# DerEchteKarsten/RayTracer3

Hardware: AMD Instinct MI355X
Metric: Mrays/s (higher is better)
Workload: dtype f32

## Files before the change

### raytracer3_amd/csrc/rt3_kernels.hip

```cpp
#include <hip/hip_fp16.h>
#include <hip/hip_runtime.h>

#include "rt3_device.hpp"
#include "rt3_internal.hpp"

namespace rt3 {

constexpr int kLdsStack = 12;
constexpr uint32_t kTopFlag = 0x40000000u;
constexpr int kSpill = 64 - kLdsStack;
constexpr uint32_t kMaxSteps = 1u << 20;

constexpr uint32_t kEmptySlot = 0xFFFFFFFFu;
constexpr float kTopPadRel = 2.44140625e-4f;

struct Cand {
    float tn;
    uint32_t ref;
};
__device__ __forceinline__ void cswap(Cand& a, Cand& b) {
    bool sw = b.tn < a.tn;
    float ta = a.tn;
    uint32_t ra = a.ref;
    a.tn = sw ? b.tn : a.tn;
// ... 314 lines not shown
                        RT3_REF48(m0, r0)
                        RT3_REF48(m1, r1)
                        RT3_REF48(m2, r2)
                        RT3_REF48(m3, r3)
#undef RT3_REF48
                    } else {
                        r0 = __float_as_uint(q2.z);
                        r1 = __float_as_uint(q2.w);
                        r2 = __float_as_uint(q3.x);
                        r3 = __float_as_uint(q3.y);
                    }
#define RT3_Q(w, b) ((float)(((w) >> (8 * (b))) & 0xFFu))
#define RT3_SLABQ(lx, ly, lz, hx, hy, hz, tn) \
    slab_test_q(__builtin_fmaf(lx, A.x, B.x), __builtin_fmaf(hx, A.x, B.x), __builtin_fmaf(ly, A.y, B.y), __builtin_fmaf(hy, A.y, B.y), \
                __builtin_fmaf(lz, A.z, B.z), __builtin_fmaf(hz, A.z, B.z), tmin, r.best.t, tn)
                    if (LAYOUT == kLayoutWide64Q) {
#define RT3_SLABS(wlo, whi, selp, selq, tn)                                                                                                    \
    (TWO ? slab_test_sorted_pad(__builtin_amdgcn_perm(whi, wlo, selp), __builtin_amdgcn_perm(whi, wlo, selq), A, B, tl_pad, tmin, r.best.t, tn) \
         : slab_test_sorted(__builtin_amdgcn_perm(whi, wlo, selp), __builtin_amdgcn_perm(whi, wlo, selq), A, B, tmin, r.best.t, tn))
                        h0 = RT3_SLABS(w0, w1, r.sel_p0, r.sel_q0, t0) & (r0 != kEmptySlot);
                        h1 = RT3_SLABS(w1, w2, r.sel_p1, r.sel_q1, t1) & (r1 != kEmptySlot);
                        h2 = RT3_SLABS(w3, w4, r.sel_p0, r.sel_q0, t2) & (r2 != kEmptySlot);
                        h3 = RT3_SLABS(w4, w5, r.sel_p1, r.sel_q1, t3) & (r3 != kEmptySlot);
#undef RT3_SLABS
                    } else {
                    h0 = RT3_SLABQ(RT3_Q(w0, 0), RT3_Q(w0, 1), RT3_Q(w0, 2), RT3_Q(w0, 3), RT3_Q(w1, 0), RT3_Q(w1, 1), t0) & (r0 != kEmptySlot);
                    h1 = RT3_SLABQ(RT3_Q(w1, 2), RT3_Q(w1, 3), RT3_Q(w2, 0), RT3_Q(w2, 1), RT3_Q(w2, 2), RT3_Q(w2, 3), t1) & (r1 != kEmptySlot);
                    h2 = RT3_SLABQ(RT3_Q(w3, 0), RT3_Q(w3, 1), RT3_Q(w3, 2), RT3_Q(w3, 3), RT3_Q(w4, 0), RT3_Q(w4, 1), t2) & (r2 != kEmptySlot);
                    h3 = RT3_SLABQ(RT3_Q(w4, 2), RT3_Q(w4, 3), RT3_Q(w5, 0), RT3_Q(w5, 1), RT3_Q(w5, 2), RT3_Q(w5, 3), t3) & (r3 != kEmptySlot);
                    }
#undef RT3_Q
#undef RT3_SLABQ
                } else {
                    r0 = __float_as_uint(q1.z);
                    r1 = __float_as_uint(q3.z);
                    r2 = __float_as_uint(q5.z);
                    r3 = __float_as_uint(q7.z);
                    h0 = slab_test_hw(v3(q0.x, q0.y, q0.z), v3(q0.w, q1.x, q1.y), o, inv, tmin, r.best.t, t0) & (r0 != kEmptySlot);
                    h1 = slab_test_hw(v3(q2.x, q2.y, q2.z), v3(q2.w, q3.x, q3.y), o, inv, tmin, r.best.t, t1) & (r1 != kEmptySlot);
                    h2 = slab_test_hw(v3(q4.x, q4.y, q4.z), v3(q4.w, q5.x, q5.y), o, inv, tmin, r.best.t, t2) & (r2 != kEmptySlot);
                    h3 = slab_test_hw(v3(q6.x, q6.y, q6.z), v3(q6.w, q7.x, q7.y), o, inv, tmin, r.best.t, t3) & (r3 != kEmptySlot);
                }
                Cand c0{h0 ? (ANY ? -t0 : t0) : kInf, h0 ? r0 : kEmptySlot}, c1{h1 ? (ANY ? -t1 : t1) : kInf, h1 ? r1 : kEmptySlot};
                Cand c2{h2 ? (ANY ? -t2 : t2) : kInf, h2 ? r2 : kEmptySlot}, c3{h3 ? (ANY ? -t3 : t3) : kInf, h3 ? r3 : kEmptySlot};
                const uint32_t nh = (uint32_t)h0 + (uint32_t)h1 + (uint32_t)h2 + (uint32_t)h3;
                cswap(c0, c1);
                cswap(c2, c3);
                cswap(c0, c2);
                cswap(c1, c3);
                cswap(c1, c2);
                if (nh > 3) {
                    if (r.sp < kLdsStack) lds[r.sp * kExtendBlock] = c3.ref;
                    else spill[r.sp - kLdsStack] = c3.ref;
                    ++r.sp;
                }
                if (nh > 2) {
                    if (r.sp < kLdsStack) lds[r.sp * kExtendBlock] = c2.ref;
                    else spill[r.sp - kLdsStack] = c2.ref;
                    ++r.sp;
                }
                if (nh > 1) {
                    if (r.sp < kLdsStack) lds[r.sp * kExtendBlock] = c1.ref;
                    else spill[r.sp - kLdsStack] = c1.ref;
                    ++r.sp;
                }
                r.cur = c0.ref;
                pop = nh == 0;
            } else {
                float tn0, tn1;
                uint32_t r0 = __float_as_uint(q3.x), r1 = __float_as_uint(q3.y);
                bool h0 = slab_test_hw(v3(q0.x, q0.y, q0.z), v3(q0.w, q1.x, q1.y), o, inv, tmin, r.best.t, tn0) & (r0 != kEmptySlot);
                bool h1 = slab_test_hw(v3(q1.z, q1.w, q2.x), v3(q2.y, q2.z, q2.w), o, inv, tmin, r.best.t, tn1) & (r1 != kEmptySlot);
                bool near1 = tn1 < tn0;
                if (h0 & h1) {
                    uint32_t far = near1 ? r0 : r1;
                    if (r.sp < kLdsStack) lds[r.sp * kExtendBlock] = far;
                    else spill[r.sp - kLdsStack] = far;
                    ++r.sp;
                }
                r.cur = (h0 & h1) ? (near1 ? r1 : r0) : (h0 ? r0 : r1);
                pop = !(h0 | h1);
            }
        }
        if (pop && !done) {
            if (TWO && tl_bottom && (uint32_t)r.sp == tl_mark) {
                tl_world();
                tl_sels();
            }
            if (r.sp == 0) {
                done = true;
            } else {
                --r.sp;
                if (r.sp < kLdsStack) {
                    r.cur = lds[r.sp * kExtendBlock];
                } else {
                    r.cur = spill[r.sp - kLdsStack];
                    __builtin_amdgcn_sched_barrier(0);
                }
            }
        }
        if (++r.steps >= kMaxSteps) done = true;
        if (done) {
            finish(r.index, r.best, r.cn, r.ct, r.cl, MODE == 2 ? lane_any : MODE == 1, r.pay0, r.pay1, r.pay2, r.pay3);
            busy = false;
        }
        }
    }
}

template <bool COUNT, int LAYOUT>
__global__ __launch_bounds__(kExtendBlock) void k_extend(const float4* __restrict__ nodes, const float4* __restrict__ tris, const float4* __restrict__ top, uint32_t n_top,
                                                         const float* __restrict__ rays, size_t stride,
                                                         const uint32_t* __restrict__ count_ptr, uint32_t count_imm,
                                                         float* __restrict__ hits, uint32_t* __restrict__ cnt_nodes,
                                                         uint32_t* __restrict__ cnt_tris, unsigned long long* __restrict__ totals,
                                                         uint32_t* __restrict__ work_counter, int payload, unsigned long long* __restrict__ lds_total) {
    __shared__ uint32_t stack[kLdsStack * kExtendBlock];
    __shared__ float4 s_top[4 * kTopNodes];
    const bool use_top = load_top(s_top, top, n_top);
    const uint32_t n = count_ptr ? *count_ptr : count_imm;
    unsigned long long tot_n = 0, tot_t = 0, tot_l = 0;
    auto finish = [&](uint32_t i, const Hit& h, uint32_t cn, uint32_t ct, uint32_t cl, bool, float, float, float, float) {
        reinterpret_cast<float4*>(hits)[i] = make_float4(h.t, h.u, h.v, __uint_as_float(h.prim));
        if (COUNT) {
            if (cnt_nodes) cnt_nodes[i] = cn;
            if (cnt_tris) cnt_tris[i] = ct;
            tot_n += cn;
            tot_t += ct;
            tot_l += cl;
        }
    };
    trace_stream<0, COUNT, LAYOUT == kLayoutTwoLevel ? kLayoutWide64Q : LAYOUT, LAYOUT == kLayoutTwoLevel>(nodes, tris, rays, stride, n, work_counter, stack + threadIdx.x, finish, false, nullptr, 0, nullptr, payload != 0, s_top, use_top);
    if (COUNT && totals) {
        atomicAdd(&totals[0], tot_n);
        atomicAdd(&totals[1], tot_t);
        if (lds_total) atomicAdd(lds_total, tot_l);
    }
}

template <bool COUNT, int LAYOUT>
__global__ __launch_bounds__(kExtendBlock) void k_shadow(const float4* __restrict__ nodes, const float4* __restrict__ tris, const float4* __restrict__ top, uint32_t n_top,
                                                         const float* __restrict__ rays, size_t stride,
                                                         const uint32_t* __restrict__ count_ptr, uint32_t count_imm,
                                                         const float* __restrict__ contrib, const uint32_t* __restrict__ pid,
                                                         float* __restrict__ lacc, size_t lstride,
                                                         uint32_t* __restrict__ occluded_out, uint32_t* __restrict__ cnt_nodes,
                                                         uint32_t* __restrict__ cnt_tris, unsigned long long* __restrict__ totals,
                                                         uint32_t* __restrict__ work_counter, unsigned long long* __restrict__ lds_total) {
    __shared__ uint32_t stack[kLdsStack * kExtendBlock];
    __shared__ float4 s_top[4 * kTopNodes];
    const bool use_top = load_top(s_top, top, n_top);
    const uint32_t n = count_ptr ? *count_ptr : count_imm;
    unsigned long long tot_n = 0, tot_t = 0, tot_l = 0;
    trace_stream<1, COUNT, LAYOUT == kLayoutTwoLevel ? kLayoutWide64Q : LAYOUT, LAYOUT == kLayoutTwoLevel>(
        nodes, tris, rays, stride, n, work_counter, stack + threadIdx.x,
        [&](uint32_t i, const Hit& h, uint32_t cn, uint32_t ct, uint32_t cl, bool, float c_r, float c_g, float c_b, float c_pid) {
            if (occluded_out) {
                occluded_out[i] = h.prim != kMiss ? 1u : 0u;
            } else if (h.prim == kMiss) {
                float4* L = reinterpret_cast<float4*>(lacc) + __float_as_uint(c_pid);
                float4 v = *L;
                *L = make_float4(v.x + c_r, v.y + c_g, v.z + c_b, 0.0f);
            }
            if (COUNT) {
                if (cnt_nodes) cnt_nodes[i] = cn;
                if (cnt_tris) cnt_tris[i] = ct;
                tot_n += cn;
                tot_t += ct;
                tot_l += cl;
            }
        },
        occluded_out == nullptr, nullptr, 0, nullptr, false, s_top, use_top, occluded_out == nullptr ? reinterpret_cast<const float2*>(contrib) : nullptr);
    if (COUNT && totals) {
        atomicAdd(&totals[0], tot_n);
        atomicAdd(&totals[1], tot_t);
        if (lds_total) atomicAdd(lds_total, tot_l);
    }
}

template <bool COUNT, int LAYOUT>
__global__ __launch_bounds__(kExtendBlock) void k_trace(const float4* __restrict__ nodes, const float4* __restrict__ tris, const float4* __restrict__ top, uint32_t n_top,
                                                        const float* __restrict__ ext_rays, const float* __restrict__ sh_rays, size_t stride,
                                                        const uint32_t* __restrict__ ext_count, const uint32_t* __restrict__ sh_count,
                                                        float* __restrict__ hits, const float* __restrict__ contrib, float* __restrict__ lacc,
                                                        unsigned long long* __restrict__ totals, uint32_t* __restrict__ work_ext,
                                                        uint32_t* __restrict__ work_sh) {
    __shared__ uint32_t stack[kLdsStack * kExtendBlock];
    __shared__ float4 s_top[4 * kTopNodes];
    const bool use_top = load_top(s_top, top, n_top);
    const uint32_t n_ext = *ext_count, n_sh = *sh_count;
    unsigned long long en = 0, et = 0, sn = 0, stt = 0, el = 0, sl = 0;
    trace_stream<2, COUNT, LAYOUT == kLayoutTwoLevel ? kLayoutWide64Q : LAYOUT, LAYOUT == kLayoutTwoLevel>(
        nodes, tris, ext_rays, stride, n_ext, work_ext, stack + threadIdx.x,
        [&](uint32_t i, const Hit& h, uint32_t cn, uint32_t ct, uint32_t cl, bool any, float c_r, float c_g, float c_b, float c_pid) {
            if (!any) {
                reinterpret_cast<float4*>(hits)[i] = make_float4(h.t, h.u, h.v, __uint_as_float(h.prim));
            } else if (h.prim == kMiss) {
                float4* L = reinterpret_cast<float4*>(lacc) + __float_as_uint(c_pid);
                float4 v = *L;
                *L = make_float4(v.x + c_r, v.y + c_g, v.z + c_b, 0.0f);
            }
            if (COUNT) {
                en += any ? 0u : cn;
                et += any ? 0u : ct;
                sn += any ? cn : 0u;
                stt += any ? ct : 0u;
                el += any ? 0u : cl;
                sl += any ? cl : 0u;
            }
        },
        true, sh_rays, n_sh, work_sh, true, s_top, use_top, reinterpret_cast<const float2*>(contrib));
    if (COUNT && totals) {
        if (blockIdx.x == 0 && threadIdx.x == 0) {
            atomicAdd(&totals[0], (unsigned long long)n_ext);
            atomicAdd(&totals[3], (unsigned long long)n_sh);
        }
        atomicAdd(&totals[1], en);
        atomicAdd(&totals[2], et);
        atomicAdd(&totals[4], sn);
        atomicAdd(&totals[5], stt);
        atomicAdd(&totals[6], el);
        atomicAdd(&totals[7], sl);
    }
}

__global__ void k_raygen(GConstDev g, const uint32_t* __restrict__ pixels, uint32_t npix, float* __restrict__ rays, size_t stride) {
    for (uint32_t i = blockIdx.x * blockDim.x + threadIdx.x; i < npix; i += gridDim.x * blockDim.x) {
        uint32_t xy = pixels[i];
        V3 o, d;
        primary_ray(g, xy & 0xFFFFu, xy >> 16, o, d);
        reinterpret_cast<float4*>(rays)[i] = make_float4(o.x, o.y, o.z, 0.0f);
        reinterpret_cast<float4*>(rays)[stride + i] = make_float4(d.x, d.y, d.z, kBackgroundDepth);
    }
}
__global__ void k_gbuffer(SceneDev sc, const uint32_t* __restrict__ pixels, uint32_t npix, uint32_t width,
                          const float* __restrict__ hits, size_t stride, uint4* __restrict__ gbuffer, float* __restrict__ depth) {
    for (uint32_t i = blockIdx.x * blockDim.x + threadIdx.x; i < npix; i += gridDim.x * blockDim.x) {
        uint32_t xy = pixels[i];
        size_t pi = (size_t)(xy >> 16) * width + (xy & 0xFFFFu);
        const float4 hrec = reinterpret_cast<const float4*>(hits)[i];
        uint32_t prim = __float_as_uint(hrec.w);
        if (prim == kMiss) {
            depth[pi] = kBackgroundDepth;
        } else {
            Surface s = hit_info(sc, prim, hrec.y, hrec.z);
            gbuffer[pi] = gbuffer_pack(s);
            depth[pi] = hrec.x;
        }
    }
}

constexpr int kShadeBlock = 512;
struct BlockAppend {
    uint32_t ext, sh;
};
__device__ __forceinline__ BlockAppend block_append2(bool want_ext, bool want_sh, unsigned long long* pair ,
                                                     uint32_t* lds ) {
    constexpr int kWaves = kShadeBlock / 64;
    const uint32_t lane = __lane_id(), wave = threadIdx.x >> 6;
    const unsigned long long m_ext = __ballot(want_ext), m_sh = __ballot(want_sh);
    if (lane == 0) {
        lds[wave] = (uint32_t)__popcll(m_ext);
        lds[kWaves + 1 + wave] = (uint32_t)__popcll(m_sh);
    }
    __syncthreads();
    if (threadIdx.x == 0) {
        uint32_t te = 0, ts = 0;
#pragma unroll
        for (int w = 0; w < kWaves; w++) {
            uint32_t ce = lds[w], cs = lds[kWaves + 1 + w];
            lds[w] = te;
            lds[kWaves + 1 + w] = ts;
            te += ce;
            ts += cs;
        }
        unsigned long long old = 0ull;
        if (te | ts) old = atomicAdd(pair, (unsigned long long)te | ((unsigned long long)ts << 32));
        lds[kWaves] = (uint32_t)old;
        lds[2 * kWaves + 1] = (uint32_t)(old >> 32);
    }
    __syncthreads();
    const unsigned long long below = (1ull << lane) - 1ull;
    BlockAppend r;
    r.ext = lds[kWaves] + lds[wave] + (uint32_t)__popcll(m_ext & below);
    r.sh = lds[2 * kWaves + 1] + lds[kWaves + 1 + wave] + (uint32_t)__popcll(m_sh & below);
    return r;
}

struct ShadeArgs {
    GConstDev g;
    SceneDev sc;
    const uint32_t* pixels;
    const uint2* pixbn;
    uint32_t npix, width;
    FastDiv npix_div;
    uint32_t s0;
    uint32_t bounce;
    const uint4* gbuffer;
    const float* depth;
    const float* in_rays;
    const float* in_hits;
    const float* in_T;
    const uint32_t* in_count;
    uint32_t n_first;
    float* out_rays;
    float* out_T;
    uint32_t* out_count;
    float* sh_rays;
    float* sh_contrib;
    uint32_t* sh_count;
    float* lacc;
    size_t stride;
};

template <bool FIRST, bool GLDS>
__global__ __launch_bounds__(kShadeBlock) __attribute__((amdgpu_waves_per_eu(6, 6))) void k_shade(ShadeArgs a) {
    __shared__ uint32_t append_lds[2][2 * (kShadeBlock / 64 + 1)];
    __shared__ ShadeGeomDev s_geoms[GLDS ? kShadeGeomsLds : 1];
    if (GLDS) {
        const uint32_t words = (a.sc.n_geoms < kShadeGeomsLds ? a.sc.n_geoms : kShadeGeomsLds) * (uint32_t)(sizeof(ShadeGeomDev) / 4);
        for (uint32_t k = threadIdx.x; k < words; k += kShadeBlock) reinterpret_cast<uint32_t*>(s_geoms)[k] = reinterpret_cast<const uint32_t*>(a.sc.shade_geoms)[k];
        __syncthreads();
    }
    uint32_t parity = 0;
    constexpr uint32_t kMargRows = 2048;
    __shared__ uint32_t s_guide_marg[kMargRows];
    __shared__ float s_cdf_marg[kMargRows + 4];
    const bool marg_in_lds = (a.g.pad[0] & RT3_FLAG_NEE_SKY) && a.sc.sky != nullptr && a.sc.sky_h <= kMargRows;
    if (marg_in_lds) {
        for (uint32_t k = threadIdx.x; k < a.sc.sky_h; k += kShadeBlock) s_guide_marg[k] = a.sc.guide_marg[k];
        for (uint32_t k = threadIdx.x; k < a.sc.sky_h + 4u; k += kShadeBlock) s_cdf_marg[k] = a.sc.cdf_marg[k];
        __syncthreads();
    }
    const float* cdf_marg = marg_in_lds ? s_cdf_marg : a.sc.cdf_marg;
    const uint32_t* guide_marg = marg_in_lds ? s_guide_marg : a.sc.guide_marg;
    const GConstDev& g = a.g;
    const uint32_t flags = g.pad[0], B = g.bounces, b = a.bounce;
    const uint32_t dims = flags ? 8u : 2u;
    const bool nee = (flags & RT3_FLAG_NEE_SKY) && a.sc.sky != nullptr;
    const bool bnz = (flags & RT3_FLAG_BLUENOISE) && a.sc.bluenoise != nullptr;
    const bool spec = (flags & RT3_FLAG_SPECULAR) != 0u;
    const size_t S = a.stride;
    const uint32_t n = FIRST ? a.n_first : *a.in_count;
    const uint32_t n_round = (n + (kShadeBlock - 1)) & ~(uint32_t)(kShadeBlock - 1);
    for (uint32_t i = blockIdx.x * blockDim.x + threadIdx.x; i < n_round; i += gridDim.x * blockDim.x) {
        bool active = i < n;
        uint32_t pid = 0;
        V3 o = v3(0, 0, 0), d = v3(0, 0, 1), T = v3(1, 1, 1);
        float t = 0.0f, pdf_b = 0.0f;
        Surface surf;
        surf.albedo = surf.emissive = v3(0, 0, 0);
        surf.normal = v3(0, 0, 1);
        surf.roughness = 1.0f;
        surf.metalness = 0.0f;
        uint32_t px = 0, py = 0, sample_in_batch = 0, bn = 0;
        HitRecord hrecord;
        hrecord.rec = make_uint4(0u, 0u, 0u, 0u);
        hrecord.prim = 0u;
        float hbu = 0.0f, hbv = 0.0f;
        float4 ro = make_float4(0.0f, 0.0f, 0.0f, 0.0f), rd = make_float4(0.0f, 0.0f, 1.0f, 0.0f);
        if (!FIRST && active) {
            ro = reinterpret_cast<const float4*>(a.in_rays)[i];
            rd = reinterpret_cast<const float4*>(a.in_rays)[S + i];
        }
        if (active) {
            pid = FIRST ? i : __float_as_uint(rd.w);
            sample_in_batch = fast_div(a.npix_div, pid);
            const uint2 pb = a.pixbn[pid - sample_in_batch * a.npix];
            px = pb.x & 0xFFFFu;
            py = pb.x >> 16;
            bn = pb.y;
        }
        if (FIRST) {
            if (active) {
                size_t pi = (size_t)py * a.width + px;
                float d0 = a.depth[pi];
                if (d0 == kBackgroundDepth) {
                    reinterpret_cast<float4*>(a.lacc)[pid] = make_float4(0.0f, 0.0f, 0.0f, 0.0f);
                    active = false;
                } else {
                    surf = gbuffer_unpack(a.gbuffer[pi]);
                    primary_ray(g, px, py, o, d);
                    t = d0;
                }
            }
        } else if (active) {
            o = v3(ro.x, ro.y, ro.z);
            d = v3(rd.x, rd.y, rd.z);
            T = v3(a.in_T[i], a.in_T[S + i], a.in_T[2 * S + i]);
            pdf_b = ro.w;
            const float4 hrec = reinterpret_cast<const float4*>(a.in_hits)[i];
            uint32_t prim = __float_as_uint(hrec.w);
            if (prim == kMiss) {
                if (nee && pdf_b > 0.0f) {
                    float su, sv;
                    direction_to_equirect_uv(d, su, sv);
                    float pl;
                    V3 rad = sky_eval_and_pdf(a.sc, su, sv, pl);
                    float w = pdf_b / (pdf_b + pl);
                    float4* Lp = reinterpret_cast<float4*>(a.lacc) + pid;
                    float4 lv = *Lp;
                    *Lp = make_float4(lv.x + T.x * (rad.x * w), lv.y + T.y * (rad.y * w), lv.z + T.z * (rad.z * w), 0.0f);
                }
                active = false;
            } else {
                t = hrec.x;
                hbu = hrec.y;
                hbv = hrec.z;
                hrecord = hit_fetch(a.sc, prim);
            }
        }
        bool emit_shadow = false, emit_ext = false;
        V3 wl = v3(0, 1, 0), contrib = v3(0, 0, 0), nd = v3(0, 0, 1), Tn = T;
        float pdf_n = 0.0f;
        if (active) {
            uint32_t seed = rng_seed(px, py, g.frame);
            uint32_t sm = a.s0 + sample_in_batch;
            uint32_t base = (sm * B + b) * dims;
            float u0 = uniform_float(seed, base), u1 = uniform_float(seed, base + 1);
            if (bnz) {
                u0 = bluenoise_shift(u0, bn & 0xFFu);
                u1 = bluenoise_shift(u1, (bn >> 8) & 0xFFu);
            }
            V3 rad = v3(0.0f, 0.0f, 0.0f);
            float pl = 0.0f, cosl = 0.0f;
            SkyPick pick;
            pick.u = pick.v = pick.sin_theta = 0.0f;
            pick.x = pick.y = 0;
            if (nee) {
                float ul0 = uniform_float(seed, base + 3), ul1 = uniform_float(seed, base + 4);
                if (bnz) {
                    ul0 = bluenoise_shift(ul0, (bn >> 16) & 0xFFu);
                    ul1 = bluenoise_shift(ul1, (bn >> 24) & 0xFFu);
                }
                pick = sky_sample_direction(a.sc, cdf_marg, guide_marg, ul0, ul1, wl);
            }
            if (!FIRST) {
                if (GLDS) surf = hit_finish(a.sc, s_geoms, hrecord, hbu, hbv);
                else surf = hit_finish(a.sc, a.sc.shade_geoms, hrecord, hbu, hbv);
            }
            V3 N = surf.normal;
            if ((flags & RT3_FLAG_FACEFORWARD) && dot(N, d) > 0.0f) N = neg(N);
            if (nee) {
                cosl = dot(N, wl);
                if (cosl > 0.0f) sky_sample_radiance(a.sc, pick, rad, pl);
            }
            V3 b1, b2;
            build_orthonormal_basis(N, b1, b2);
            V3 wi = v3(0.0f, 0.0f, 1.0f), vop = surf.albedo, wo = v3(0.0f, 0.0f, 1.0f);
            float pdf_s = 0.0f;
            bool valid = true;
            Bsdf bs;
            const bool last = b == B - 1;
            if (spec) {
                bs = bsdf_setup(surf.albedo, surf.roughness, surf.metalness);
                wo = v3(-(d.x * b1.x + d.y * b1.y + d.z * b1.z), -(d.x * b2.x + d.y * b2.y + d.z * b2.z), -(d.x * N.x + d.y * N.y + d.z * N.z));
                if (!last) {
                    float u2 = uniform_float(seed, base + 2);
                    valid = bsdf_sample(bs, wo, u0, u1, u2, wi, vop, pdf_s);
                }
            } else if (!last) {
                wi = diffuse_sample(u0, u1);
                pdf_s = wi.z * kInvPi;
            }
            o = v3(o.x + t * d.x, o.y + t * d.y, o.z + t * d.z);
            if (FIRST) {
                reinterpret_cast<float4*>(a.lacc)[pid] = make_float4(T.x * surf.emissive.x, T.y * surf.emissive.y, T.z * surf.emissive.z, 0.0f);
            } else if (surf.emissive.x != 0.0f || surf.emissive.y != 0.0f || surf.emissive.z != 0.0f) {
                float4* Lp = reinterpret_cast<float4*>(a.lacc) + pid;
                float4 lv = *Lp;
                *Lp = make_float4(lv.x + T.x * surf.emissive.x, lv.y + T.y * surf.emissive.y, lv.z + T.z * surf.emissive.z, 0.0f);
            }
            if (nee) {
                if (cosl > 0.0f && pl > 0.0f) {
                    V3 fv;
                    float scale;
                    if (spec) {
                        float pproj;
                        bsdf_eval(bs, wo, v3(dot(wl, b1), dot(wl, b2), cosl), fv, pproj);
                        float pb = pproj * cosl;
                        scale = (b == B - 1) ? cosl / pl : cosl / (pl + pb);
                    } else {
                        float pb = cosl * kInvPi;
                        fv = surf.albedo;
                        scale = (b == B - 1) ? (cosl * kInvPi) / pl : (cosl * kInvPi) / (pl + pb);
                    }
                    contrib = v3((T.x * fv.x) * (rad.x * scale), (T.y * fv.y) * (rad.y * scale), (T.z * fv.z) * (rad.z * scale));
                    emit_shadow = true;
                }
            }
            if (valid && !last) {
                nd = basis_apply(b1, b2, N, wi);
                pdf_n = pdf_s;
                Tn = T * vop;
                emit_ext = true;
            }
        }
        const BlockAppend slot = block_append2(emit_ext, emit_shadow, reinterpret_cast<unsigned long long*>(a.out_count), append_lds[parity]);
        parity ^= 1u;
        if (emit_shadow) {
            const uint32_t j = slot.sh;
            reinterpret_cast<float4*>(a.sh_rays)[j] = make_float4(o.x, o.y, o.z, contrib.x);
            reinterpret_cast<float4*>(a.sh_rays)[S + j] = make_float4(wl.x, wl.y, wl.z, contrib.y);
            reinterpret_cast<float2*>(a.sh_contrib)[j] = make_float2(contrib.z, __uint_as_float(pid));
        }
        if (emit_ext) {
            const uint32_t j = slot.ext;
            reinterpret_cast<float4*>(a.out_rays)[j] = make_float4(o.x, o.y, o.z, pdf_n);
            reinterpret_cast<float4*>(a.out_rays)[S + j] = make_float4(nd.x, nd.y, nd.z, __uint_as_float(pid));
            a.out_T[j] = Tn.x;
            a.out_T[S + j] = Tn.y;
            a.out_T[2 * S + j] = Tn.z;
        }
    }
}

__global__ void k_accumulate(GConstDev g, const uint32_t* __restrict__ pixels, uint32_t npix, uint32_t width,
                             const float* __restrict__ depth, const float* __restrict__ lacc, size_t stride, uint32_t sb,
                             int first_batch, int last_batch, float* __restrict__ radsum, float4* __restrict__ light,
                             const float4* __restrict__ prev) {
    for (uint32_t i = blockIdx.x * blockDim.x + threadIdx.x; i < npix; i += gridDim.x * blockDim.x) {
        uint32_t xy = pixels[i];
        size_t pi = (size_t)(xy >> 16) * width + (xy & 0xFFFFu);
        if (depth[pi] == kBackgroundDepth) continue;
        float r = first_batch ? 0.0f : radsum[i], gg = first_batch ? 0.0f : radsum[npix + i], bb = first_batch ? 0.0f : radsum[2 * (size_t)npix + i];
        for (uint32_t s = 0; s < sb; s++) {
            size_t p = (size_t)s * npix + i;
            const float4 lv = reinterpret_cast<const float4*>(lacc)[p];
            r += lv.x;
            gg += lv.y;
            bb += lv.z;
        }
        if (!last_batch) {
            radsum[i] = r;
            radsum[npix + i] = gg;
            radsum[2 * (size_t)npix + i] = bb;
        } else {
            float fs = (float)g.samples;
            r = r / fs;
            gg = gg / fs;
            bb = bb / fs;
            if (g.blendfactor >= 1.0f) {
                light[pi] = make_float4(r, gg, bb, 0.0f);
            } else {
                float4 pv = prev[pi];
                float bf = g.blendfactor;
                light[pi] = make_float4(pv.x + (r - pv.x) * bf, pv.y + (gg - pv.y) * bf, pv.z + (bb - pv.z) * bf, 0.0f);
            }
        }
    }
}

__device__ __forceinline__ float agx_contrast(float x) {
    float x2 = x * x, x4 = x2 * x2;
    return 15.5f * x4 * x2 - 40.14f * x4 * x + 31.96f * x4 - 6.868f * x2 * x + 0.4298f * x2 + 0.1191f * x - 0.00232f;
}
__device__ __forceinline__ V3 agx_tonemap(V3 c) {
    const float m[9] = {0.842479062253094f, 0.0423282422610123f, 0.0423756549057051f, 0.0784335999999992f, 0.878468636469772f,
                        0.0784336f, 0.0792237451477643f, 0.0791661274605434f, 0.879142973793104f};
    const float mi[9] = {1.19687900512017f, -0.0528968517574562f, -0.0529716355144438f, -0.0980208811401368f, 1.15190312990417f,
                         -0.0980434501171241f, -0.0990297440797205f, -0.0989611768448433f, 1.15107367264116f};
    const float min_ev = -12.47393f, max_ev = 4.026069f;
    float v[3], w[3];
#pragma unroll
    for (int j = 0; j < 3; j++) v[j] = c.x * m[j] + c.y * m[3 + j] + c.z * m[6 + j];
#pragma unroll
    for (int j = 0; j < 3; j++) {
        float l = v[j] > 0.0f ? log2f(v[j]) : min_ev;
        l = fmin_sel(fmax_sel(l, min_ev), max_ev);
        l = (l - min_ev) / (max_ev - min_ev);
        v[j] = agx_contrast(l);
    }
    float luma = v[0] * 0.2126f + v[1] * 0.7152f + v[2] * 0.0722f;
#pragma unroll
    for (int j = 0; j < 3; j++) w[j] = luma + 1.1f * (powf(fmax_sel(v[j], 0.0f), 1.1f) - luma);
    return v3(w[0] * mi[0] + w[1] * mi[3] + w[2] * mi[6], w[0] * mi[1] + w[1] * mi[4] + w[2] * mi[7], w[0] * mi[2] + w[1] * mi[5] + w[2] * mi[8]);
}
__global__ void k_postprocess(GConstDev g, SceneDev sc, const uint32_t* __restrict__ pixels, uint32_t npix, uint32_t width,
                              const float* __restrict__ depth, const float4* __restrict__ in, float4* __restrict__ out) {
    for (uint32_t i = blockIdx.x * blockDim.x + threadIdx.x; i < npix; i += gridDim.x * blockDim.x) {
        uint32_t xy = pixels[i], px = xy & 0xFFFFu, py = xy >> 16;
        size_t pi = (size_t)py * width + px;
        V3 col;
        if (depth[pi] != kBackgroundDepth) {
            float4 c = in[pi];
            col = v3(c.x, c.y, c.z);
        } else {
            V3 o, d;
            primary_ray(g, px, py, o, d);
            float su, sv;
            direction_to_equirect_uv(d, su, sv);
            col = sky_eval(sc, su, sv);
        }
        V3 r = agx_tonemap(col);
        out[pi] = make_float4(r.x, r.y, r.z, 1.0f);
    }
}

__global__ void k_pack_tiles(const uint32_t* __restrict__ pixels, uint32_t npix, uint32_t width, const float4* __restrict__ img,
                             float4* __restrict__ dst) {
    for (uint32_t i = blockIdx.x * blockDim.x + threadIdx.x; i < npix; i += gridDim.x * blockDim.x) {
        uint32_t xy = pixels[i];
        dst[i] = img[(size_t)(xy >> 16) * width + (xy & 0xFFFFu)];
    }
}
__global__ void k_unpack_tiles(const uint32_t* __restrict__ pixels, uint32_t npix, uint32_t width, const float4* __restrict__ src,
                               float4* __restrict__ img) {
    for (uint32_t i = blockIdx.x * blockDim.x + threadIdx.x; i < npix; i += gridDim.x * blockDim.x) {
        uint32_t xy = pixels[i];
        img[(size_t)(xy >> 16) * width + (xy & 0xFFFFu)] = src[i];
    }
}

__global__ void k_selftest(int op, const uint32_t* __restrict__ in, uint32_t n, uint32_t* __restrict__ out) {
    uint32_t i = blockIdx.x * blockDim.x + threadIdx.x;
    if (i >= n) return;
    auto F = [](uint32_t u) { return __uint_as_float(u); };
    auto U = [](float f) { return __float_as_uint(f); };
    switch (op) {
        case 0: out[i] = jenkins_hash(in[i]); break;
        case 1: out[i] = zcurve(in[2 * i], in[2 * i + 1]); break;
        case 2: out[i] = murmur3(in[2 * i], in[2 * i + 1]); break;
        case 3: out[i] = U(uniform_float(in[2 * i], in[2 * i + 1])); break;
        case 4: {
            const uint32_t* p = in + 11 * i;
            Surface s;
            s.albedo = v3(F(p[0]), F(p[1]), F(p[2]));
            s.emissive = v3(F(p[3]), F(p[4]), F(p[5]));
            s.normal = v3(F(p[6]), F(p[7]), F(p[8]));
            s.roughness = F(p[9]);
            s.metalness = F(p[10]);
            uint4 q = gbuffer_pack(s);
            out[4 * i] = q.x; out[4 * i + 1] = q.y; out[4 * i + 2] = q.z; out[4 * i + 3] = q.w;
            break;
        }
        case 5: {
            Surface s = gbuffer_unpack(make_uint4(in[4 * i], in[4 * i + 1], in[4 * i + 2], in[4 * i + 3]));
            uint32_t* o = out + 11 * i;
            o[0] = U(s.albedo.x); o[1] = U(s.albedo.y); o[2] = U(s.albedo.z);
            o[3] = U(s.emissive.x); o[4] = U(s.emissive.y); o[5] = U(s.emissive.z);
            o[6] = U(s.normal.x); o[7] = U(s.normal.y); o[8] = U(s.normal.z);
            o[9] = U(s.roughness); o[10] = U(s.metalness);
            break;
        }
        case 6: {
            V3 w = diffuse_sample(F(in[2 * i]), F(in[2 * i + 1]));
            out[3 * i] = U(w.x); out[3 * i + 1] = U(w.y); out[3 * i + 2] = U(w.z);
            break;
        }
        case 7: {
            V3 b1, b2;
            build_orthonormal_basis(v3(F(in[3 * i]), F(in[3 * i + 1]), F(in[3 * i + 2])), b1, b2);
            uint32_t* o = out + 6 * i;
            o[0] = U(b1.x); o[1] = U(b1.y); o[2] = U(b1.z); o[3] = U(b2.x); o[4] = U(b2.y); o[5] = U(b2.z);
            break;
        }
        case 8: {
            V3 r = agx_tonemap(v3(F(in[3 * i]), F(in[3 * i + 1]), F(in[3 * i + 2])));
            out[3 * i] = U(r.x); out[3 * i + 1] = U(r.y); out[3 * i + 2] = U(r.z);
            break;
        }
        case 9: {
            float sn, cs;
            sincos_2pi(F(in[i]), sn, cs);
            out[2 * i] = U(sn); out[2 * i + 1] = U(cs);
            break;
        }
        case 10: out[i] = U(atan2_poly(F(in[2 * i]), F(in[2 * i + 1]))); break;
        case 11: out[i] = rng_seed(in[3 * i], in[3 * i + 1], in[3 * i + 2]); break;
        case 12: {
            const uint32_t nn = in[2 * i], dd = in[2 * i + 1];
            const FastDiv f = make_fastdiv(dd);
            const uint32_t q = fast_div(f, nn);
            out[3 * i] = q;
            out[3 * i + 1] = nn - q * dd;
            out[3 * i + 2] = (uint32_t)wrap_index((int)nn, (int)(dd & 0xFFFFu) + 1);
            break;
        }
        case 17: out[i] = octa_encode16(v3(F(in[3 * i]), F(in[3 * i + 1]), F(in[3 * i + 2]))); break;
        case 18: {
            const V3 n = octa_decode16(in[i]);
            out[3 * i] = U(n.x);
            out[3 * i + 1] = U(n.y);
            out[3 * i + 2] = U(n.z);
            break;
        }
        default: break;
    }
}
bool selftest_widths(int op, uint32_t* in_w, uint32_t* out_w) {
    static const uint32_t w[19][2] = {{1, 1}, {2, 1}, {2, 1}, {2, 1}, {11, 4}, {4, 11}, {2, 3}, {3, 6}, {3, 3}, {1, 2}, {2, 1}, {3, 1}, {2, 3},
                                      {2, 3}, {3, 9}, {64, 128}, {64, 1}, {3, 1}, {1, 3}};
    if (op < 0 || op > 18) return false;
    *in_w = w[op][0];
    *out_w = w[op][1];
    return true;
}
void launch_selftest(hipStream_t st, int op, const uint32_t* in, uint32_t n, uint32_t* out) {
    if (op >= 13 && op <= 16) return launch_selftest_probes(st, op, in, n, out);
    hipLaunchKernelGGL(k_selftest, dim3((n + 255) / 256), dim3(256), 0, st, op, in, n, out);
}

static inline unsigned grid_for(uint64_t n, unsigned block, unsigned max_blocks) {
    uint64_t b = (n + block - 1) / block;
    if (b < 1) b = 1;
    return (unsigned)(b > max_blocks ? max_blocks : b);
}

void launch_raygen(hipStream_t st, const GConstDev& g, const uint32_t* pixels, uint32_t npix, float* rays, size_t stride) {
    hipLaunchKernelGGL(k_raygen, dim3(grid_for(npix, 256, 4096)), dim3(256), 0, st, g, pixels, npix, rays, stride);
}
void launch_extend(hipStream_t st, bool count, int layout, const float4* nodes, const float4* tris, const float4* top, uint32_t n_top, const float* rays, size_t stride,
                   const uint32_t* count_ptr, uint32_t count_imm, uint32_t max_n, float* hits, uint32_t* cn, uint32_t* ct,
                   unsigned long long* totals, uint32_t* work_counter, bool payload) {
    unsigned grid = grid_for(max_n, kExtendBlock, g_trace_max_blocks);
#define RT3_LAUNCH_EXTEND(C, L)                                                                                                                  \
    hipLaunchKernelGGL((k_extend<C, L>), dim3(grid), dim3(kExtendBlock), 0, st, nodes, tris, top, n_top, rays, stride, count_ptr, count_imm, hits, cn, ct, totals, \
                       work_counter, payload ? 1 : 0, totals ? totals + 10 : nullptr )
    if (count) {
        if (layout == kLayoutTwoLevel) RT3_LAUNCH_EXTEND(true, kLayoutTwoLevel);
        else if (layout == kLayoutWide48Q) RT3_LAUNCH_EXTEND(true, kLayoutWide48Q);
        else if (layout == kLayoutWide64Q) RT3_LAUNCH_EXTEND(true, kLayoutWide64Q);
        else if (layout == kLayoutWide128) RT3_LAUNCH_EXTEND(true, kLayoutWide128);
        else RT3_LAUNCH_EXTEND(true, kLayoutBinary64);
    } else {
        if (layout == kLayoutTwoLevel) RT3_LAUNCH_EXTEND(false, kLayoutTwoLevel);
        else if (layout == kLayoutWide48Q) RT3_LAUNCH_EXTEND(false, kLayoutWide48Q);
        else if (layout == kLayoutWide64Q) RT3_LAUNCH_EXTEND(false, kLayoutWide64Q);
        else if (layout == kLayoutWide128) RT3_LAUNCH_EXTEND(false, kLayoutWide128);
        else RT3_LAUNCH_EXTEND(false, kLayoutBinary64);
    }
#undef RT3_LAUNCH_EXTEND
}
void launch_shadow(hipStream_t st, bool count, int layout, const float4* nodes, const float4* tris, const float4* top, uint32_t n_top, const float* rays, size_t stride,
                   const uint32_t* count_ptr, uint32_t count_imm, uint32_t max_n, const float* contrib, const uint32_t* pid, float* lacc,
                   size_t lstride, uint32_t* occluded_out, uint32_t* cn, uint32_t* ct, unsigned long long* totals, uint32_t* work_counter) {
    unsigned grid = grid_for(max_n, kExtendBlock, g_trace_max_blocks);
#define RT3_LAUNCH_SHADOW(C, L)                                                                                                                \
    hipLaunchKernelGGL((k_shadow<C, L>), dim3(grid), dim3(kExtendBlock), 0, st, nodes, tris, top, n_top, rays, stride, count_ptr, count_imm, contrib, pid, lacc, \
                       lstride, occluded_out, cn, ct, totals, work_counter, totals ? totals + 9 : nullptr )
    if (count) {
        if (layout == kLayoutTwoLevel) RT3_LAUNCH_SHADOW(true, kLayoutTwoLevel);
        else if (layout == kLayoutWide48Q) RT3_LAUNCH_SHADOW(true, kLayoutWide48Q);
        else if (layout == kLayoutWide64Q) RT3_LAUNCH_SHADOW(true, kLayoutWide64Q);
        else if (layout == kLayoutWide128) RT3_LAUNCH_SHADOW(true, kLayoutWide128);
        else RT3_LAUNCH_SHADOW(true, kLayoutBinary64);
    } else {
        if (layout == kLayoutTwoLevel) RT3_LAUNCH_SHADOW(false, kLayoutTwoLevel);
        else if (layout == kLayoutWide48Q) RT3_LAUNCH_SHADOW(false, kLayoutWide48Q);
        else if (layout == kLayoutWide64Q) RT3_LAUNCH_SHADOW(false, kLayoutWide64Q);
        else if (layout == kLayoutWide128) RT3_LAUNCH_SHADOW(false, kLayoutWide128);
        else RT3_LAUNCH_SHADOW(false, kLayoutBinary64);
    }
#undef RT3_LAUNCH_SHADOW
}
void launch_trace(hipStream_t st, bool count, int layout, const float4* nodes, const float4* tris, const float4* top, uint32_t n_top, const float* ext_rays, const float* sh_rays,
                  size_t stride, const uint32_t* ext_count, const uint32_t* sh_count, uint32_t max_n, float* hits, const float* contrib, float* lacc,
                  unsigned long long* totals, uint32_t* work_ext, uint32_t* work_sh) {
    unsigned grid = grid_for(max_n, kExtendBlock, g_trace_max_blocks);
#define RT3_LAUNCH_TRACE(C, L)                                                                                                                  \
    hipLaunchKernelGGL((k_trace<C, L>), dim3(grid), dim3(kExtendBlock), 0, st, nodes, tris, top, n_top, ext_rays, sh_rays, stride, ext_count, sh_count, hits, \
                       contrib, lacc, totals, work_ext, work_sh)
    if (count) {
        if (layout == kLayoutTwoLevel) RT3_LAUNCH_TRACE(true, kLayoutTwoLevel);
        else if (layout == kLayoutWide48Q) RT3_LAUNCH_TRACE(true, kLayoutWide48Q);
        else if (layout == kLayoutWide64Q) RT3_LAUNCH_TRACE(true, kLayoutWide64Q);
        else if (layout == kLayoutWide128) RT3_LAUNCH_TRACE(true, kLayoutWide128);
        else RT3_LAUNCH_TRACE(true, kLayoutBinary64);
    } else {
        if (layout == kLayoutTwoLevel) RT3_LAUNCH_TRACE(false, kLayoutTwoLevel);
        else if (layout == kLayoutWide48Q) RT3_LAUNCH_TRACE(false, kLayoutWide48Q);
        else if (layout == kLayoutWide64Q) RT3_LAUNCH_TRACE(false, kLayoutWide64Q);
        else if (layout == kLayoutWide128) RT3_LAUNCH_TRACE(false, kLayoutWide128);
        else RT3_LAUNCH_TRACE(false, kLayoutBinary64);
    }
#undef RT3_LAUNCH_TRACE
}
void launch_gbuffer(hipStream_t st, const SceneDev& sc, const uint32_t* pixels, uint32_t npix, uint32_t width, const float* hits,
                    size_t stride, void* gbuffer, float* depth) {
    hipLaunchKernelGGL(k_gbuffer, dim3(grid_for(npix, 256, 4096)), dim3(256), 0, st, sc, pixels, npix, width, hits, stride, (uint4*)gbuffer, depth);
}
__global__ void k_pixbn(const uint32_t* __restrict__ pixels, uint32_t npix, const uint8_t* __restrict__ bluenoise, uint32_t bn_w, uint32_t bn_h,
                        uint2* __restrict__ out) {
    for (uint32_t i = blockIdx.x * blockDim.x + threadIdx.x; i < npix; i += gridDim.x * blockDim.x) {
        const uint32_t xy = pixels[i], px = xy & 0xFFFFu, py = xy >> 16;
        uint32_t bn = 0;
        if (bluenoise) bn = *reinterpret_cast<const uint32_t*>(bluenoise + 4 * ((size_t)(py % bn_h) * bn_w + (px % bn_w)));
        out[i] = make_uint2(xy, bn);
    }
}
void launch_pixbn(hipStream_t st, const uint32_t* pixels, uint32_t npix, const uint8_t* bluenoise, uint32_t bn_w, uint32_t bn_h, uint2* out) {
    hipLaunchKernelGGL(k_pixbn, dim3(grid_for(npix, 256, 4096)), dim3(256), 0, st, pixels, npix, bluenoise, bn_w, bn_h, out);
}
void launch_shade(hipStream_t st, bool first, const ShadeLaunch& L) {
    ShadeArgs a;
    a.g = L.g; a.sc = L.sc; a.pixels = L.pixels; a.npix = L.npix; a.width = L.width; a.s0 = L.s0; a.bounce = L.bounce;
    a.npix_div = make_fastdiv(L.npix);
    a.pixbn = L.pixbn;
    a.gbuffer = (const uint4*)L.gbuffer; a.depth = L.depth;
    a.in_rays = L.in_rays; a.in_hits = L.in_hits; a.in_T = L.in_T; a.in_count = L.in_count; a.n_first = L.n_first;
    a.out_rays = L.out_rays; a.out_T = L.out_T; a.out_count = L.out_count;
    a.sh_rays = L.sh_rays; a.sh_contrib = L.sh_contrib; a.sh_count = L.sh_count;
    a.lacc = L.lacc; a.stride = L.stride;
    unsigned grid = grid_for(L.max_n, kShadeBlock, 8192);
    if (first) hipLaunchKernelGGL((k_shade<true, false>), dim3(grid), dim3(kShadeBlock), 0, st, a);
    else if (a.sc.shade_geoms != nullptr && a.sc.n_geoms <= kShadeGeomsLds) hipLaunchKernelGGL((k_shade<false, true>), dim3(grid), dim3(kShadeBlock), 0, st, a);
    else hipLaunchKernelGGL((k_shade<false, false>), dim3(grid), dim3(kShadeBlock), 0, st, a);
}
void launch_accumulate(hipStream_t st, const GConstDev& g, const uint32_t* pixels, uint32_t npix, uint32_t width, const float* depth,
                       const float* lacc, size_t stride, uint32_t sb, int first_batch, int last_batch, float* radsum, void* light,
                       const void* prev) {
    hipLaunchKernelGGL(k_accumulate, dim3(grid_for(npix, 256, 8192)), dim3(256), 0, st, g, pixels, npix, width, depth, lacc, stride, sb,
                       first_batch, last_batch, radsum, (float4*)light, (const float4*)prev);
}
void launch_postprocess(hipStream_t st, const GConstDev& g, const SceneDev& sc, const uint32_t* pixels, uint32_t npix, uint32_t width,
                        const float* depth, const void* in, void* out) {
    hipLaunchKernelGGL(k_postprocess, dim3(grid_for(npix, 256, 8192)), dim3(256), 0, st, g, sc, pixels, npix, width, depth, (const float4*)in,
                       (float4*)out);
}
void launch_pack_tiles(hipStream_t st, const uint32_t* pixels, uint32_t npix, uint32_t width, const void* img, void* dst) {
    hipLaunchKernelGGL(k_pack_tiles, dim3(grid_for(npix, 256, 8192)), dim3(256), 0, st, pixels, npix, width, (const float4*)img, (float4*)dst);
}
void launch_unpack_tiles(hipStream_t st, const uint32_t* pixels, uint32_t npix, uint32_t width, const void* src, void* img) {
    hipLaunchKernelGGL(k_unpack_tiles, dim3(grid_for(npix, 256, 8192)), dim3(256), 0, st, pixels, npix, width, (const float4*)src, (float4*)img);
}

}
```

Measured before the change: 7590.

## Amortize first-bounce per-pixel setup across runs of samples in shade kernel

The first-vertex shading path now gives each thread one pixel and loops over up to eight samples of that pixel. Per-pixel work (gbuffer unpack, depth read, primary ray, basis build, BSDF setup, RNG seed) is done once per run instead of once per sample, and the per-sample fast division and pixbn lookup are gone. The launch grid is resized to cover pixel-block times sample-run units. This costs more live registers and longer serial loops per thread, and it changes the order of appended rays, which can affect coherence in later bounces.

```diff
diff --git a/raytracer3_amd/csrc/rt3_kernels.hip b/raytracer3_amd/csrc/rt3_kernels.hip
--- a/raytracer3_amd/csrc/rt3_kernels.hip
+++ b/raytracer3_amd/csrc/rt3_kernels.hip
@@ -640,7 +640,7 @@
     const float* in_hits;
     const float* in_T;
     const uint32_t* in_count;
-    uint32_t n_first;
+    uint32_t sb;
     float* out_rays;
     float* out_T;
     uint32_t* out_count;
@@ -651,6 +651,145 @@
     size_t stride;
 };
 
+constexpr uint32_t kFirstRun = 8;
+__device__ __forceinline__ void shade_first_vertex(const ShadeArgs& a, const float* cdf_marg, const uint32_t* guide_marg, uint32_t (*append_lds)[2 * (kShadeBlock / 64 + 1)]) {
+    const GConstDev& g = a.g;
+    const uint32_t flags = g.pad[0], B = g.bounces, b = a.bounce;
+    const uint32_t dims = flags ? 8u : 2u;
+    const bool nee = (flags & RT3_FLAG_NEE_SKY) && a.sc.sky != nullptr;
+    const bool bnz = (flags & RT3_FLAG_BLUENOISE) && a.sc.bluenoise != nullptr;
+    const bool spec = (flags & RT3_FLAG_SPECULAR) != 0u;
+    const bool last = b == B - 1;
+    const size_t S = a.stride;
+    const uint32_t npix = a.npix, n_pb = (npix + (kShadeBlock - 1)) / kShadeBlock, n_units = n_pb * ((a.sb + (kFirstRun - 1)) / kFirstRun);
+    uint32_t parity = 0;
+    for (uint32_t unit = blockIdx.x; unit < n_units; unit += gridDim.x) {
+        const uint32_t run = unit / n_pb, p = (unit - run * n_pb) * kShadeBlock + threadIdx.x;
+        const uint32_t s_end = min((run + 1) * kFirstRun, a.sb);
+        bool active = p < npix, background = false;
+        const V3 T = v3(1, 1, 1);
+        V3 o = v3(0, 0, 0), d = v3(0, 0, 1);
+        float t = 0.0f;
+        Surface surf;
+        surf.albedo = surf.emissive = v3(0, 0, 0);
+        surf.normal = v3(0, 0, 1);
+        surf.roughness = 1.0f;
+        surf.metalness = 0.0f;
+        uint32_t px = 0, py = 0, bn = 0;
+        if (active) {
+            const uint2 pb = a.pixbn[p];
+            px = pb.x & 0xFFFFu;
+            py = pb.x >> 16;
+            bn = pb.y;
+            size_t pi = (size_t)py * a.width + px;
+            float d0 = a.depth[pi];
+            if (d0 == kBackgroundDepth) {
+                background = true;
+                active = false;
+            } else {
+                surf = gbuffer_unpack(a.gbuffer[pi]);
+                primary_ray(g, px, py, o, d);
+                t = d0;
+            }
+        }
+        uint32_t seed = 0;
+        V3 N = surf.normal, b1 = v3(1, 0, 0), b2 = v3(0, 1, 0), wo = v3(0.0f, 0.0f, 1.0f);
+        Bsdf bs;
+        if (active) {
+            seed = rng_seed(px, py, g.frame);
+            if ((flags & RT3_FLAG_FACEFORWARD) && dot(N, d) > 0.0f) N = neg(N);
+            build_orthonormal_basis(N, b1, b2);
+            if (spec) {
+                bs = bsdf_setup(surf.albedo, surf.roughness, surf.metalness);
+                wo = v3(-(d.x * b1.x + d.y * b1.y + d.z * b1.z), -(d.x * b2.x + d.y * b2.y + d.z * b2.z), -(d.x * N.x + d.y * N.y + d.z * N.z));
+            }
+            o = v3(o.x + t * d.x, o.y + t * d.y, o.z + t * d.z);
+        }
+        for (uint32_t s = run * kFirstRun; s < s_end; s++) {
+            const uint32_t pid = s * npix + p;
+            asm volatile("" : "+v"(wo.x), "+v"(wo.y), "+v"(wo.z), "+v"(bs.alpha), "+v"(bs.p_spec), "+v"(bn));
+            if (background) reinterpret_cast<float4*>(a.lacc)[pid] = make_float4(0.0f, 0.0f, 0.0f, 0.0f);
+            bool emit_shadow = false, emit_ext = false;
+            V3 wl = v3(0, 1, 0), contrib = v3(0, 0, 0), nd = v3(0, 0, 1), Tn = T;
+            float pdf_n = 0.0f;
+            if (active) {
+                uint32_t sm = a.s0 + s;
+                uint32_t base = (sm * B + b) * dims;
+                float u0 = uniform_float(seed, base), u1 = uniform_float(seed, base + 1);
+                if (bnz) {
+                    u0 = bluenoise_shift(u0, bn & 0xFFu);
+                    u1 = bluenoise_shift(u1, (bn >> 8) & 0xFFu);
+                }
+                V3 rad = v3(0.0f, 0.0f, 0.0f);
+                float pl = 0.0f, cosl = 0.0f;
+                if (nee) {
+                    float ul0 = uniform_float(seed, base + 3), ul1 = uniform_float(seed, base + 4);
+                    if (bnz) {
+                        ul0 = bluenoise_shift(ul0, (bn >> 16) & 0xFFu);
+                        ul1 = bluenoise_shift(ul1, (bn >> 24) & 0xFFu);
+                    }
+                    const SkyPick pick = sky_sample_direction(a.sc, cdf_marg, guide_marg, ul0, ul1, wl);
+                    cosl = dot(N, wl);
+                    if (cosl > 0.0f) sky_sample_radiance(a.sc, pick, rad, pl);
+                }
+                V3 wi = v3(0.0f, 0.0f, 1.0f), vop = surf.albedo;
+                float pdf_s = 0.0f;
+                bool valid = true;
+                if (spec) {
+                    if (!last) {
+                        float u2 = uniform_float(seed, base + 2);
+                        valid = bsdf_sample(bs, wo, u0, u1, u2, wi, vop, pdf_s);
+                    }
+                } else if (!last) {
+                    wi = diffuse_sample(u0, u1);
+                    pdf_s = wi.z * kInvPi;
+                }
+                reinterpret_cast<float4*>(a.lacc)[pid] = make_float4(T.x * surf.emissive.x, T.y * surf.emissive.y, T.z * surf.emissive.z, 0.0f);
+                if (nee) {
+                    if (cosl > 0.0f && pl > 0.0f) {
+                        V3 fv;
+                        float scale;
+                        if (spec) {
+                            float pproj;
+                            bsdf_eval(bs, wo, v3(dot(wl, b1), dot(wl, b2), cosl), fv, pproj);
+                            float pb = pproj * cosl;
+                            scale = (b == B - 1) ? cosl / pl : cosl / (pl + pb);
+                        } else {
+                            float pb = cosl * kInvPi;
+                            fv = surf.albedo;
+                            scale = (b == B - 1) ? (cosl * kInvPi) / pl : (cosl * kInvPi) / (pl + pb);
+                        }
+                        contrib = v3((T.x * fv.x) * (rad.x * scale), (T.y * fv.y) * (rad.y * scale), (T.z * fv.z) * (rad.z * scale));
+                        emit_shadow = true;
+                    }
+                }
+                if (valid && !last) {
+                    nd = basis_apply(b1, b2, N, wi);
+                    pdf_n = pdf_s;
+                    Tn = T * vop;
+                    emit_ext = true;
+                }
+            }
+            const BlockAppend slot = block_append2(emit_ext, emit_shadow, reinterpret_cast<unsigned long long*>(a.out_count), append_lds[parity]);
+            parity ^= 1u;
+            if (emit_shadow) {
+                const uint32_t j = slot.sh;
+                reinterpret_cast<float4*>(a.sh_rays)[j] = make_float4(o.x, o.y, o.z, contrib.x);
+                reinterpret_cast<float4*>(a.sh_rays)[S + j] = make_float4(wl.x, wl.y, wl.z, contrib.y);
+                reinterpret_cast<float2*>(a.sh_contrib)[j] = make_float2(contrib.z, __uint_as_float(pid));
+            }
+            if (emit_ext) {
+                const uint32_t j = slot.ext;
+                reinterpret_cast<float4*>(a.out_rays)[j] = make_float4(o.x, o.y, o.z, pdf_n);
+                reinterpret_cast<float4*>(a.out_rays)[S + j] = make_float4(nd.x, nd.y, nd.z, __uint_as_float(pid));
+                a.out_T[j] = Tn.x;
+                a.out_T[S + j] = Tn.y;
+                a.out_T[2 * S + j] = Tn.z;
+            }
+        }
+    }
+}
+
 template <bool FIRST, bool GLDS>
 __global__ __launch_bounds__(kShadeBlock) __attribute__((amdgpu_waves_per_eu(6, 6))) void k_shade(ShadeArgs a) {
     __shared__ uint32_t append_lds[2][2 * (kShadeBlock / 64 + 1)];
@@ -679,7 +818,11 @@
     const bool bnz = (flags & RT3_FLAG_BLUENOISE) && a.sc.bluenoise != nullptr;
     const bool spec = (flags & RT3_FLAG_SPECULAR) != 0u;
     const size_t S = a.stride;
-    const uint32_t n = FIRST ? a.n_first : *a.in_count;
+    if constexpr (FIRST) {
+        shade_first_vertex(a, cdf_marg, guide_marg, append_lds);
+        return;
+    }
+    const uint32_t n = *a.in_count;
     const uint32_t n_round = (n + (kShadeBlock - 1)) & ~(uint32_t)(kShadeBlock - 1);
     for (uint32_t i = blockIdx.x * blockDim.x + threadIdx.x; i < n_round; i += gridDim.x * blockDim.x) {
         bool active = i < n;
@@ -697,32 +840,19 @@
         hrecord.prim = 0u;
         float hbu = 0.0f, hbv = 0.0f;
         float4 ro = make_float4(0.0f, 0.0f, 0.0f, 0.0f), rd = make_float4(0.0f, 0.0f, 1.0f, 0.0f);
-        if (!FIRST && active) {
+        if (active) {
             ro = reinterpret_cast<const float4*>(a.in_rays)[i];
             rd = reinterpret_cast<const float4*>(a.in_rays)[S + i];
         }
         if (active) {
-            pid = FIRST ? i : __float_as_uint(rd.w);
+            pid = __float_as_uint(rd.w);
             sample_in_batch = fast_div(a.npix_div, pid);
             const uint2 pb = a.pixbn[pid - sample_in_batch * a.npix];
             px = pb.x & 0xFFFFu;
             py = pb.x >> 16;
             bn = pb.y;
         }
-        if (FIRST) {
-            if (active) {
-                size_t pi = (size_t)py * a.width + px;
-                float d0 = a.depth[pi];
-                if (d0 == kBackgroundDepth) {
-                    reinterpret_cast<float4*>(a.lacc)[pid] = make_float4(0.0f, 0.0f, 0.0f, 0.0f);
-                    active = false;
-                } else {
-                    surf = gbuffer_unpack(a.gbuffer[pi]);
-                    primary_ray(g, px, py, o, d);
-                    t = d0;
-                }
-            }
-        } else if (active) {
+        if (active) {
             o = v3(ro.x, ro.y, ro.z);
             d = v3(rd.x, rd.y, rd.z);
             T = v3(a.in_T[i], a.in_T[S + i], a.in_T[2 * S + i]);
@@ -773,10 +903,8 @@
                 }
                 pick = sky_sample_direction(a.sc, cdf_marg, guide_marg, ul0, ul1, wl);
             }
-            if (!FIRST) {
-                if (GLDS) surf = hit_finish(a.sc, s_geoms, hrecord, hbu, hbv);
-                else surf = hit_finish(a.sc, a.sc.shade_geoms, hrecord, hbu, hbv);
-            }
+            if (GLDS) surf = hit_finish(a.sc, s_geoms, hrecord, hbu, hbv);
+            else surf = hit_finish(a.sc, a.sc.shade_geoms, hrecord, hbu, hbv);
             V3 N = surf.normal;
             if ((flags & RT3_FLAG_FACEFORWARD) && dot(N, d) > 0.0f) N = neg(N);
             if (nee) {
@@ -802,9 +930,7 @@
                 pdf_s = wi.z * kInvPi;
             }
             o = v3(o.x + t * d.x, o.y + t * d.y, o.z + t * d.z);
-            if (FIRST) {
-                reinterpret_cast<float4*>(a.lacc)[pid] = make_float4(T.x * surf.emissive.x, T.y * surf.emissive.y, T.z * surf.emissive.z, 0.0f);
-            } else if (surf.emissive.x != 0.0f || surf.emissive.y != 0.0f || surf.emissive.z != 0.0f) {
+            if (surf.emissive.x != 0.0f || surf.emissive.y != 0.0f || surf.emissive.z != 0.0f) {
                 float4* Lp = reinterpret_cast<float4*>(a.lacc) + pid;
                 float4 lv = *Lp;
                 *Lp = make_float4(lv.x + T.x * surf.emissive.x, lv.y + T.y * surf.emissive.y, lv.z + T.z * surf.emissive.z, 0.0f);
@@ -1136,13 +1262,15 @@
     a.npix_div = make_fastdiv(L.npix);
     a.pixbn = L.pixbn;
     a.gbuffer = (const uint4*)L.gbuffer; a.depth = L.depth;
-    a.in_rays = L.in_rays; a.in_hits = L.in_hits; a.in_T = L.in_T; a.in_count = L.in_count; a.n_first = L.n_first;
+    a.in_rays = L.in_rays; a.in_hits = L.in_hits; a.in_T = L.in_T; a.in_count = L.in_count; a.sb = L.n_first / L.npix;
     a.out_rays = L.out_rays; a.out_T = L.out_T; a.out_count = L.out_count;
     a.sh_rays = L.sh_rays; a.sh_contrib = L.sh_contrib; a.sh_count = L.sh_count;
     a.lacc = L.lacc; a.stride = L.stride;
     unsigned grid = grid_for(L.max_n, kShadeBlock, 8192);
-    if (first) hipLaunchKernelGGL((k_shade<true, false>), dim3(grid), dim3(kShadeBlock), 0, st, a);
-    else if (a.sc.shade_geoms != nullptr && a.sc.n_geoms <= kShadeGeomsLds) hipLaunchKernelGGL((k_shade<false, true>), dim3(grid), dim3(kShadeBlock), 0, st, a);
+    if (first) {
+        const uint64_t units = (uint64_t)((L.npix + kShadeBlock - 1) / kShadeBlock) * ((a.sb + kFirstRun - 1) / kFirstRun);
+        hipLaunchKernelGGL((k_shade<true, false>), dim3(grid_for(units, 1, 8192)), dim3(kShadeBlock), 0, st, a);
+    } else if (a.sc.shade_geoms != nullptr && a.sc.n_geoms <= kShadeGeomsLds) hipLaunchKernelGGL((k_shade<false, true>), dim3(grid), dim3(kShadeBlock), 0, st, a);
     else hipLaunchKernelGGL((k_shade<false, false>), dim3(grid), dim3(kShadeBlock), 0, st, a);
 }
 void launch_accumulate(hipStream_t st, const GConstDev& g, const uint32_t* pixels, uint32_t npix, uint32_t width, const float* depth,
```

Result: faster. 7723 (median of 6 runs) (+1.8%).
